# Westlake-AGI-Lab/WorldForge

Measured on AMD Instinct MI355X. Metric: denoising steps/sec (81f x 480p, Wan2.1-14B), higher is better.
Workload: dtype bf16

## Files before the change

### include/wf_hip.h

```cpp
#ifndef WF_HIP_H_
#define WF_HIP_H_

#include <stddef.h>
#include <stdint.h>

#ifdef __cplusplus
extern "C" {
#endif

#define WF_OK 0
#define WF_EINVAL (-1)
#define WF_EHIP (-2)
#define WF_ENOTSUP (-3)

#define WF_F32 0
#define WF_BF16 1

int wf_version(void);
const char* wf_last_error(void);
int wf_device_info(int dev, int* n_cu, int* clock_khz, char* name, int name_len);


int wf_cfg_combine(const void* cond, const void* uncond, void* out, int dt, float g, size_t n, void* stream);

// ... 57 lines not shown
int wf_gemm_f16_batched(const void* X, const void* W, void* out, int batch, int M, int N, int K, int ldx, int ldw, int ldo, int64_t bsx,
                        int64_t bsw, int64_t bso, int epilogue, void* stream);
int wf_mx_quant_e4m3(const void* X, void* Q, void* S, int M, int K, int ldx, void* stream);
int wf_gemm_mxfp8(const void* Xq, const void* Xs, const void* Wq, const void* Ws, const float* bias, void* out, const float* gate, int M, int N,
                  int K, int ldx, int ldw, int ldo, int epilogue, void* stream);
int wf_lora_fold(const void* base, void* out, int N, int K, int n_adapters, const void* U0, const void* D0, int rank0, int nsep0,
                 float scale0, const void* U1, const void* D1, int rank1, int nsep1, float scale1, const void* U2, const void* D2,
                 int rank2, int nsep2, float scale2, const void* U3, const void* D3, int rank3, int nsep3, float scale3, void* stream);

int wf_attn_fwd(const void* Q, const void* K, const void* Vt, void* O, int H, int Lq, int Lkp, int kv_len, int seg_len,
                size_t seg_stride_bytes, int ldo, float softmax_scale, int accumulate, const float* kmax2, int kmax_n, int kmax_stride,
                const float* qmax2, int qmax_n, void* stream);
int wf_head_max_norm2(const void* X, int H, int L, int Lp, float* out, void* stream);
size_t wf_attn_split_workspace_bytes(int H, int Lq, int nsplit);
int wf_attn_cross2_fwd(const void* Q, const void* K, const void* Vt, void* O, int H, int Lq, int Lk1p, int kv_len1, int Lk2p, int kv_len2,
                       int ldo, float softmax_scale, void* stream);
int wf_attn_debug_body_counter(void* counters2);
int wf_attn_fwd_split(const void* Q, const void* K, const void* Vt, void* O, int H, int Lq, int Lkp, int kv_len, int seg_len,
                      size_t seg_stride_bytes, int ldo, float softmax_scale, int accumulate, int nsplit, void* workspace, const float* kmax2,
                      int kmax_n, int kmax_stride, const float* qmax2, int qmax_n, void* stream);
int wf_attn_fwd_part(const void* Q, const void* K, const void* Vt, int H, int Lq, int Lkp, int kv_len, int seg_len, size_t seg_stride_bytes,
                     int t_begin, int t_end, int t_begin2, int t_end2, int inner_splits, int part, int nparts, void* workspace, void* O_merge,
                     int ldo, const float* kmax2, int kmax_n, int kmax_stride, const float* qmax2, int qmax_n, void* stream);
int wf_attn_merge(void* O, int H, int Lq, int ldo, int accumulate, int nparts, const void* workspace, void* stream);

int wf_ln_modulate(const float* x, const float* mul, const float* add, void* out, int out_dtype, int L, int C, float eps,
                   int plus_one, void* stream);

int wf_rmsnorm_heads(const void* in, int ld, const float* weight, const float* cos_tab, const float* sin_tab, void* out, int L,
                     int Lout, int C, float eps, float out_scale, void* stream);
size_t wf_rmsnorm_heads_bound_ws_floats(int L, int C);
int wf_rmsnorm_heads_bound(const void* in, int ld, const float* weight, const float* cos_tab, const float* sin_tab, void* out, int L, int Lout,
                           int C, float eps, float out_scale, float* ws, float* max_norm2, void* stream);

int wf_v_transpose(const void* V, int ld, void* Vt, int L, int Lp, int H, void* stream);
int wf_v_transpose_seg(const void* V, int ld, void* Vt, int L, int Lp, int H, int head_stride_tiles, void* stream);
int wf_v_transpose_at(const void* V, int ld, void* Vt, int k0, int L, int Lp, int H, void* stream);

int wf_patchify(const void* x, void* tokens, int Cin, int T, int Hh, int Ww, void* stream);
int wf_unpatchify(const float* y, float* out, int Cout, int T, int Hh, int Ww, void* stream);

int wf_act(const void* a, int dt_a, const void* b, int dt_b, void* out, int dt_out, int mode, size_t n, void* stream);

int wf_lc_ln_modulate(const void* x, const float* mul, const float* add, int64_t mod_ld, int rows_per_group, int64_t row0,
                      const int* group_index, int plus_one, void* out, int L, int C, float eps, void* stream);
int wf_lc_gate_residual(void* x, const void* y, int64_t ldy, const float* gate, int64_t gate_ld, int rows_per_group, int64_t row0,
                        const int* group_index, int L, int C, void* stream);
int wf_lc_norm_heads(const void* in, int64_t ld, const float* weight, const float* cos_tab, const float* sin_tab, void* out, int L,
                     int Lout, int H, float eps, float out_scale, void* stream);
int wf_lc_swiglu(const void* in, int64_t ld, void* out, int L, int Hd, void* stream);

int wf_refine_upsample_u8(const void* frames_u8, float* out, int F, int H0, int W0, int Fo, int H, int W, void* stream);

int wf_lc_mean_pool_blocks(const void* in, void* out, int H, int L, int block, void* stream);
int wf_lc_mean_pool_blocks_at(const void* in, int64_t in_head_stride_rows, void* out, int out_head_stride_blocks, int b0, int H, int L,
                              int block, void* stream);
int wf_bsa_topk_lists(const void* scores, int64_t ld, int heads, int n_q, int n_k, int n_sel, int block, int blocks_per_segment,
                      int* lists, int* counts, int max_entries, uint32_t* sel_mask, void* stream);
int wf_bsa_cdf_lists(const void* scores, int64_t ld, int heads, int n_q, int n_k, float cdf_threshold, int n_min, int block,
                     int blocks_per_segment, int* lists, int* counts, int max_entries, uint32_t* sel_mask, int* row_counts, void* stream);
int wf_gather_rows_bf16(const void* in, int64_t ld_in, const int* index, void* out, int64_t ld_out, int n_rows, int C, void* stream);
int wf_attn_bsa_fwd(const void* Q, const void* K, const void* Vt, void* O, int H, int Lq, int Lkp, int seg_len, int ldo,
                    float softmax_scale, const int* group_lists, const int* group_counts, int max_entries, int block, void* stream);

int wf_t5_attn_fwd(const void* Q, const void* K, const void* V, int ldqkv, void* O, int ldo, const float* bias, const void* bucket_lut,
                   int lmax, int num_buckets, int H, int L, int kv_len, void* stream);
// ... 122 lines not shown
```

### worldforge_amd/csrc/dit_ops.hip

```cpp
#include "common.h"
#include "mfma.h"

using namespace wf;

namespace {

__device__ __forceinline__ float block_sum_1(float v, float* sm, int nwaves) {
  v = wave_sum(v);
  const int lane = threadIdx.x & 63, wid = threadIdx.x >> 6;
  __syncthreads();
  if (lane == 0) sm[wid] = v;
  __syncthreads();
  float t = 0.f;
  for (int i = 0; i < nwaves; ++i) t += sm[i];
  return t;
}

template <int VPT>
__global__ __launch_bounds__(256) void k_ln_mod(const float* __restrict__ x, const float* __restrict__ mul,
                                                const float* __restrict__ add, void* __restrict__ out, int out_bf16, int C,
                                                float eps, float plus_one) {
  __shared__ float sm[8];
  const size_t row = blockIdx.x;
  const float4* xr = reinterpret_cast<const float4*>(x + row * C);
  const int nvec = C >> 2;
  float4 v[VPT];
  float s = 0.f;
#pragma unroll
  for (int i = 0; i < VPT; ++i) {
    int id = threadIdx.x + 256 * i;
    if (id < nvec) {
      v[i] = xr[id];
      s += (v[i].x + v[i].y) + (v[i].z + v[i].w);
    } else {
      v[i] = make_float4(0.f, 0.f, 0.f, 0.f);
    }
  }
  const float mean = block_sum_1(s, sm, 4) / (float)C;
  float q = 0.f;
#pragma unroll
  for (int i = 0; i < VPT; ++i) {
    int id = threadIdx.x + 256 * i;
    if (id < nvec) {
      float a = v[i].x - mean, b = v[i].y - mean, c = v[i].z - mean, d = v[i].w - mean;
      q += (a * a + b * b) + (c * c + d * d);
    }
  }
  const float var = block_sum_1(q, sm, 4) / (float)C;
  const float rstd = rsqrtf(var + eps);
#pragma unroll
  for (int i = 0; i < VPT; ++i) {
    int id = threadIdx.x + 256 * i;
    if (id < nvec) {
      float4 m4 = mul ? reinterpret_cast<const float4*>(mul)[id] : make_float4(0.f, 0.f, 0.f, 0.f);
      float4 a4 = add ? reinterpret_cast<const float4*>(add)[id] : make_float4(0.f, 0.f, 0.f, 0.f);
      float y0 = (v[i].x - mean) * rstd * (plus_one + m4.x) + a4.x;
      float y1 = (v[i].y - mean) * rstd * (plus_one + m4.y) + a4.y;
      float y2 = (v[i].z - mean) * rstd * (plus_one + m4.z) + a4.z;
      float y3 = (v[i].w - mean) * rstd * (plus_one + m4.w) + a4.w;
      if (out_bf16) {
        u32x2 pk = {pack_bf16x2(y0, y1), pack_bf16x2(y2, y3)};
        reinterpret_cast<u32x2*>(reinterpret_cast<uint16_t*>(out) + row * C)[id] = pk;
      } else {
        reinterpret_cast<float4*>(reinterpret_cast<float*>(out) + row * C)[id] = make_float4(y0, y1, y2, y3);
      }
    }
  }
}

__global__ __launch_bounds__(128) void k_rms_heads(const uint16_t* __restrict__ in, int ld, const float* __restrict__ w,
                                                   const float* __restrict__ cs, const float* __restrict__ sn,
                                                   uint16_t* __restrict__ out, int L, int Lout, int C, float eps, float out_scale,
                                                   float* __restrict__ norm2_rows) {
  __shared__ float sm[4];
  const int row = blockIdx.x;
  const uint16_t* xr = in + (size_t)row * ld;
  const int nch = C >> 3;
  constexpr int MAXC = 8;
  u32x4 v[MAXC];
  float ss = 0.f;
#pragma unroll
  for (int i = 0; i < MAXC; ++i) {
    int id = threadIdx.x + 128 * i;
    if (id < nch) {
      v[i] = reinterpret_cast<const u32x4*>(xr)[id];
#pragma unroll
      for (int k = 0; k < 4; ++k) {
        float a = __uint_as_float(v[i][k] << 16), b = __uint_as_float(v[i][k] & 0xffff0000u);
        ss += a * a + b * b;
      }
    }
  }
  const float tot = block_sum_1(ss, sm, 2);
  const float rinv = rsqrtf(tot / (float)C + eps);
  const int H = C >> 7;
#pragma unroll
  for (int i = 0; i < MAXC; ++i) {
    int id = threadIdx.x + 128 * i;
    if (id < nch) {
      const int head = id >> 4, within = id & 15;
      const float4 w0 = reinterpret_cast<const float4*>(w)[2 * id], w1 = reinterpret_cast<const float4*>(w)[2 * id + 1];
      const float ww[8] = {w0.x, w0.y, w0.z, w0.w, w1.x, w1.y, w1.z, w1.w};
      float y[8];
#pragma unroll
      for (int k = 0; k < 4; ++k) {
        float a = __uint_as_float(v[i][k] << 16), b = __uint_as_float(v[i][k] & 0xffff0000u);
        y[2 * k] = rbf(rbf(a * rinv) * ww[2 * k]);
        y[2 * k + 1] = rbf(rbf(b * rinv) * ww[2 * k + 1]);
      }
      if (cs) {
        const float4 c4 = reinterpret_cast<const float4*>(cs + (size_t)row * 64)[within];
        const float4 s4 = reinterpret_cast<const float4*>(sn + (size_t)row * 64)[within];
        const float cc[4] = {c4.x, c4.y, c4.z, c4.w}, sv[4] = {s4.x, s4.y, s4.z, s4.w};
#pragma unroll
        for (int k = 0; k < 4; ++k) {
          float re = y[2 * k] * cc[k] - y[2 * k + 1] * sv[k];
          float im = y[2 * k] * sv[k] + y[2 * k + 1] * cc[k];
          y[2 * k] = re;
          y[2 * k + 1] = im;
        }
      }
      if (out_scale != 1.0f) {
#pragma unroll
        for (int k = 0; k < 8; ++k) y[k] *= out_scale;
      }
      u32x4 pk = {pack_bf16x2(y[0], y[1]), pack_bf16x2(y[2], y[3]), pack_bf16x2(y[4], y[5]), pack_bf16x2(y[6], y[7])};
      *reinterpret_cast<u32x4*>(out + ((size_t)head * Lout + row) * 128 + within * 8) = pk;
      if (norm2_rows) {
        float q = 0.f;
#pragma unroll
        for (int k = 0; k < 4; ++k) {
          const float a = __uint_as_float(pk[k] << 16), b = __uint_as_float(pk[k] & 0xffff0000u);
          q += a * a + b * b;
        }
        q += __shfl_xor(q, 8, 64);
        q += __shfl_xor(q, 4, 64);
        q += __shfl_xor(q, 2, 64);
        q += __shfl_xor(q, 1, 64);
        if (within == 0) norm2_rows[(size_t)row * H + head] = q;
      }
    }
  }
}

constexpr int NB_RB = 128;
__device__ __forceinline__ float nb_max(float best, float v) { return !(v <= 3.0e38f) ? INFINITY : fmaxf(best, v); }
__device__ __forceinline__ float nb_column_max(const float* __restrict__ src, int n, int H, int h, int s, int ns) {
  float best = 0.f;
  int r = s;
  for (; r + 7 * ns < n; r += 8 * ns) {
    float v[8];
#pragma unroll
    for (int u = 0; u < 8; ++u) v[u] = src[(size_t)(r + u * ns) * H + h];
#pragma unroll
    for (int u = 0; u < 8; ++u) best = nb_max(best, v[u]);
  }
  for (; r < n; r += ns) best = nb_max(best, src[(size_t)r * H + h]);
  return best;
}
__global__ __launch_bounds__(256) void k_norm2_part(const float* __restrict__ rows, int L, int H, float* __restrict__ part) {
  __shared__ float red[256];
  const int t = threadIdx.x, h = t % H, s = t / H, ns = 256 / H;
  const int r0 = blockIdx.x * NB_RB, n = min(L - r0, NB_RB);
  float best = s < ns ? nb_column_max(rows + (size_t)r0 * H, n, H, h, s, ns) : 0.f;
  red[t] = best;
  __syncthreads();
  if (t < H) {
    for (int k = 1; k < ns; ++k) best = fmaxf(best, red[k * H + t]);
    part[(size_t)blockIdx.x * H + t] = best;
  }
}
__global__ __launch_bounds__(256) void k_norm2_final(const float* __restrict__ part, int nblk, int H, float* __restrict__ out) {
  __shared__ float red[256];
  const int t = threadIdx.x, h = t % H, s = t / H, ns = 256 / H;
  float best = s < ns ? nb_column_max(part, nblk, H, h, s, ns) : 0.f;
// ... 2 lines not shown
  if (t < H) {
    for (int k = 1; k < ns; ++k) best = fmaxf(best, red[k * H + t]);
    out[t] = best;
  }
}

__global__ __launch_bounds__(256) void k_vt(const uint16_t* __restrict__ V, int ld, uint16_t* __restrict__ Vt, int L, int hstride) {
  __shared__ uint16_t tile[64][136];
  const int kt = blockIdx.x, head = blockIdx.y;
  const int tid = threadIdx.x;
#pragma unroll
  for (int i = 0; i < 4; ++i) {
    int id = tid + 256 * i;
    int r = id >> 4, c = id & 15;
    int key = kt * 64 + r;
    u32x4 v = {0u, 0u, 0u, 0u};
    if (key < L) v = *reinterpret_cast<const u32x4*>(V + (size_t)key * ld + head * 128 + c * 8);
    *reinterpret_cast<u32x4*>(&tile[r][c * 8]) = v;
  }
  __syncthreads();
  uint16_t* dst = Vt + ((size_t)head * hstride + kt) * (128 * 64);
#pragma unroll
  for (int i = 0; i < 4; ++i) {
    int id = tid + 256 * i;
    int d = id >> 3, c = id & 7;
    uint32_t p[4];
#pragma unroll
    for (int k = 0; k < 4; ++k) p[k] = (uint32_t)tile[c * 8 + 2 * k][d] | ((uint32_t)tile[c * 8 + 2 * k + 1][d] << 16);
    u32x4 pk = {p[0], p[1], p[2], p[3]};
    *reinterpret_cast<u32x4*>(dst + d * 64 + c * 8) = pk;
  }
}

__global__ void k_patchify(const uint16_t* __restrict__ x, uint16_t* __restrict__ out, int Cin, int T, int Hh, int Ww, size_t n) {
  const int h2 = Hh >> 1, w2 = Ww >> 1, K = Cin * 4;
  for (size_t i = (size_t)blockIdx.x * blockDim.x + threadIdx.x; i < n; i += (size_t)gridDim.x * blockDim.x) {
    int k = (int)(i % K);
    size_t tok = i / K;
    int c = k >> 2, ph = (k >> 1) & 1, pw = k & 1;
    int wx = (int)(tok % w2), hy = (int)((tok / w2) % h2), f = (int)(tok / ((size_t)w2 * h2));
    out[i] = x[(((size_t)c * T + f) * Hh + (2 * hy + ph)) * Ww + (2 * wx + pw)];
  }
}
__global__ void k_unpatchify(const float* __restrict__ y, float* __restrict__ out, int Cout, int T, int Hh, int Ww, size_t n) {
  const int h2 = Hh >> 1, w2 = Ww >> 1;
  for (size_t i = (size_t)blockIdx.x * blockDim.x + threadIdx.x; i < n; i += (size_t)gridDim.x * blockDim.x) {
    int xw = (int)(i % Ww), yh = (int)((i / Ww) % Hh), f = (int)((i / ((size_t)Ww * Hh)) % T), c = (int)(i / ((size_t)Ww * Hh * T));
    size_t tok = ((size_t)f * h2 + (yh >> 1)) * w2 + (xw >> 1);
    int k = (((yh & 1) << 1) | (xw & 1)) * Cout + c;
    out[i] = y[tok * (4 * Cout) + k];
  }
}

__global__ void k_act(TView a, TView b, TView o, int mode, size_t n) {
  for (size_t i = (size_t)blockIdx.x * blockDim.x + threadIdx.x; i < n; i += (size_t)gridDim.x * blockDim.x) {
    float v = tload(a, i);
    if (b.p) v += tload(b, i);
    if (mode == 0)
      v = v / (1.0f + __expf(-v));
    else if (mode == 1)
      v = 0.5f * v * (1.0f + erff(v * 0.70710678118654752f));
    tstore(o, i, v);
  }
}

}

extern "C" int wf_ln_modulate(const float* x, const float* mul, const float* add, void* out, int out_dtype, int L, int C,
                              float eps, int plus_one, void* stream) {
  WF_CHECK_ARG(x && out, "wf_ln_modulate: null pointer");
  WF_CHECK_ARG(C % 4 == 0 && C <= 8192 && C > 0, "wf_ln_modulate: C=%d must be a multiple of 4 and <= 8192", C);
  if (L == 0) return WF_OK;
  hipStream_t s = (hipStream_t)stream;
  const float p1 = plus_one ? 1.0f : 0.0f;
  const int ob = out_dtype == WF_BF16;
  const int nvec = C / 4;
  if (nvec <= 512)
    hipLaunchKernelGGL(k_ln_mod<2>, dim3(L), dim3(256), 0, s, x, mul, add, out, ob, C, eps, p1);
  else if (nvec <= 1280)
    hipLaunchKernelGGL(k_ln_mod<5>, dim3(L), dim3(256), 0, s, x, mul, add, out, ob, C, eps, p1);
  else
    hipLaunchKernelGGL(k_ln_mod<8>, dim3(L), dim3(256), 0, s, x, mul, add, out, ob, C, eps, p1);
  WF_LAUNCH_CHECK("wf_ln_modulate");
  return WF_OK;
}

extern "C" int wf_rmsnorm_heads(const void* in, int ld, const float* weight, const float* cos_tab, const float* sin_tab,
                                void* out, int L, int Lout, int C, float eps, float out_scale, void* stream) {
  WF_CHECK_ARG(in && weight && out, "wf_rmsnorm_heads: null pointer");
  WF_CHECK_ARG(out_scale > 0.0f, "wf_rmsnorm_heads: out_scale must be positive (1 = none)");
  WF_CHECK_ARG(C % 128 == 0 && C <= 8192 && ld % 8 == 0, "wf_rmsnorm_heads: C=%d must be a multiple of 128 (<= 8192), ld %% 8", C);
  WF_CHECK_ARG(Lout >= L, "wf_rmsnorm_heads: Lout < L");
  WF_CHECK_ARG((cos_tab == nullptr) == (sin_tab == nullptr), "wf_rmsnorm_heads: cos/sin must both be given or both null");
  if (L == 0) return WF_OK;
  hipLaunchKernelGGL(k_rms_heads, dim3(L), dim3(128), 0, (hipStream_t)stream, (const uint16_t*)in, ld, weight, cos_tab,
                     sin_tab, (uint16_t*)out, L, Lout, C, eps, out_scale, (float*)nullptr);
  WF_LAUNCH_CHECK("wf_rmsnorm_heads");
  return WF_OK;
}

extern "C" size_t wf_rmsnorm_heads_bound_ws_floats(int L, int C) {
  if (L <= 0 || C <= 0) return 0;
  const size_t H = (size_t)C / 128;
  return (size_t)L * H + (size_t)((L + NB_RB - 1) / NB_RB) * H;
}

extern "C" int wf_rmsnorm_heads_bound(const void* in, int ld, const float* weight, const float* cos_tab, const float* sin_tab, void* out,
                                      int L, int Lout, int C, float eps, float out_scale, float* ws, float* max_norm2, void* stream) {
  WF_CHECK_ARG(in && weight && out && ws && max_norm2, "wf_rmsnorm_heads_bound: null pointer");
  WF_CHECK_ARG(out_scale > 0.0f, "wf_rmsnorm_heads_bound: out_scale must be positive (1 = none)");
  WF_CHECK_ARG(C >= 128 && C % 128 == 0 && C <= 8192 && ld % 8 == 0, "wf_rmsnorm_heads_bound: C=%d must be a multiple of 128 in 128..8192, ld %% 8", C);
  WF_CHECK_ARG(Lout >= L && L > 0, "wf_rmsnorm_heads_bound: need 0 < L <= Lout");
  WF_CHECK_ARG((cos_tab == nullptr) == (sin_tab == nullptr), "wf_rmsnorm_heads_bound: cos/sin must both be given or both null");
  const int H = C / 128, nblk = (L + NB_RB - 1) / NB_RB;
  float* rows = ws;
  float* part = ws + (size_t)L * H;
  hipLaunchKernelGGL(k_rms_heads, dim3(L), dim3(128), 0, (hipStream_t)stream, (const uint16_t*)in, ld, weight, cos_tab,
                     sin_tab, (uint16_t*)out, L, Lout, C, eps, out_scale, rows);
  hipLaunchKernelGGL(k_norm2_part, dim3(nblk), dim3(256), 0, (hipStream_t)stream, rows, L, H, part);
  hipLaunchKernelGGL(k_norm2_final, dim3(1), dim3(256), 0, (hipStream_t)stream, part, nblk, H, max_norm2);
  WF_LAUNCH_CHECK("wf_rmsnorm_heads_bound");
  return WF_OK;
}

extern "C" int wf_v_transpose(const void* V, int ld, void* Vt, int L, int Lp, int H, void* stream) {
  WF_CHECK_ARG(V && Vt, "wf_v_transpose: null pointer");
  WF_CHECK_ARG(Lp % 64 == 0 && Lp >= L && ld % 8 == 0, "wf_v_transpose: Lp must be a multiple of 64 and >= L");
  if (Lp == 0) return WF_OK;
  hipLaunchKernelGGL(k_vt, dim3(Lp / 64, H), dim3(256), 0, (hipStream_t)stream, (const uint16_t*)V, ld, (uint16_t*)Vt, L, Lp / 64);
  WF_LAUNCH_CHECK("wf_v_transpose");
  return WF_OK;
}

extern "C" int wf_v_transpose_seg(const void* V, int ld, void* Vt, int L, int Lp, int H, int head_stride_tiles, void* stream) {
  WF_CHECK_ARG(V && Vt, "wf_v_transpose_seg: null pointer");
  WF_CHECK_ARG(Lp % 64 == 0 && Lp >= L && ld % 8 == 0, "wf_v_transpose_seg: Lp must be a multiple of 64 and >= L");
  WF_CHECK_ARG(head_stride_tiles >= Lp / 64, "wf_v_transpose_seg: head stride (%d tiles) shorter than the segment (%d)", head_stride_tiles, Lp / 64);
  if (Lp == 0) return WF_OK;
  hipLaunchKernelGGL(k_vt, dim3(Lp / 64, H), dim3(256), 0, (hipStream_t)stream, (const uint16_t*)V, ld, (uint16_t*)Vt, L, head_stride_tiles);
  WF_LAUNCH_CHECK("wf_v_transpose_seg");
  return WF_OK;
}

extern "C" int wf_patchify(const void* x, void* tokens, int Cin, int T, int Hh, int Ww, void* stream) {
  WF_CHECK_ARG(x && tokens, "wf_patchify: null pointer");
  WF_CHECK_ARG(Hh % 2 == 0 && Ww % 2 == 0, "wf_patchify: latent H, W must be even");
  size_t n = (size_t)T * (Hh / 2) * (Ww / 2) * Cin * 4;
  if (n == 0) return WF_OK;
  hipLaunchKernelGGL(k_patchify, dim3(grid_for(n, 256, 4096)), dim3(256), 0, (hipStream_t)stream, (const uint16_t*)x,
                     (uint16_t*)tokens, Cin, T, Hh, Ww, n);
  WF_LAUNCH_CHECK("wf_patchify");
  return WF_OK;
}

// ... 20 lines not shown
```

### worldforge_amd/dit.py

```python
from __future__ import annotations

import math
import os
from dataclasses import dataclass
from types import SimpleNamespace
from typing import Dict, Optional, Tuple

import numpy as np
import torch

from . import _ffi, ops
from ._ffi import WF_BF16, WF_F32, call
from .forward_common import (ForwardWorkspaces, GatheredLayerKV, act, bf16_latents, gather_layer_kv, layers_per_rank, run,
                             seeded_generators)

EPI_BF16, EPI_BF16_GELU, EPI_F32, EPI_RESID, EPI_F32_ACC = 0, 1, 2, 3, 4


@dataclass
class DiTConfig:
    dim: int = 5120
    ffn_dim: int = 13824
    num_heads: int = 40
    num_layers: int = 40
# ... 52 lines not shown
    out = dict(W)
    for k, v in W.items():
        if k.endswith(tuple(suffixes)):
            out[k] = MXWeight.quantize(v)
    return out


def gemm(x: torch.Tensor, w, bias: Optional[torch.Tensor], out: torch.Tensor, epi: int,
         gate: Optional[torch.Tensor] = None):
    if isinstance(w, MXWeight):
        xq, xs = _mx_act(x)
        return ops.gemm_mxfp8(xq, xs, w.q, w.s, bias, out, epi, gate)
    M, K = x.shape
    N = w.shape[0]
    assert w.shape[1] == K and x.dtype == torch.bfloat16 and w.dtype == torch.bfloat16
    assert out.shape[0] == M and out.shape[1] == N
    call("wf_gemm_bf16", x.data_ptr(), w.data_ptr(), bias.data_ptr() if bias is not None else None, out.data_ptr(),
         gate.data_ptr() if gate is not None else None, M, N, K, x.stride(0), w.stride(0), out.stride(0), epi, ops.stream())
    return out


def ffn_padded_features(f: int) -> int:
    fp = -(-f // 320) * 320
    return fp if (fp - f) * 100 <= 3 * f else f


def _pad_rows(t: torch.Tensor, rows: int) -> torch.Tensor:
    if t.shape[0] == rows:
        return t
    pad = torch.zeros((rows - t.shape[0],) + tuple(t.shape[1:]), dtype=t.dtype, device=t.device)
    return torch.cat([t, pad], 0).contiguous()


PROFILE_ATTN = None
PROFILE_COMM = None


def comm_wait_ms(entry) -> float:
    if isinstance(entry, list):
        return sum(a.elapsed_time(b) for a, b in entry)
    return entry[0].elapsed_time(entry[1])


def kv_splits(H: int, Lq: int, kv_len: int, n_cu: int = 256) -> int:
    if kv_len < 128 * 64:
        return 1
    w = -(-Lq // 256) * H
    eff = lambda n: (w * n / n_cu) / -(-(w * n) // n_cu)
    return 2 if eff(2) > eff(1) + 0.08 else 1


def head_max_norm2(k: torch.Tensor, L: int, out: torch.Tensor) -> torch.Tensor:
    H, Lp, _ = k.shape
    out.zero_()
    call("wf_head_max_norm2", k.data_ptr(), H, L, Lp, out.data_ptr(), ops.stream())
    return out


def attention(q: torch.Tensor, k: torch.Tensor, vt: torch.Tensor, out: torch.Tensor, kv_len: int, scale: float,
              accumulate: bool = False, profile: bool = False, nsplit: Optional[int] = None, kmax2: Optional[torch.Tensor] = None,
              qmax2: Optional[torch.Tensor] = None):
    H, Lq, D = q.shape
    seg_stride = 0
    if k.dim() == 4:
        P, _, seg, _ = k.shape
        assert vt.shape == (P, H, seg // 64, 128, 64)
# ... 595 lines not shown
        ws.hbuf = _buf("h", (L, d), bf)
        ws.qkv = _buf("qkv", (L, 3 * d), bf)
        ws.qh = _buf("qh", (H, L, 128), bf)
        ws.qm = _buf("qmax2", (H,), f32) if pl.use_bounds else None
        if pl.exchange is not None:
            ws.ex = self._exchange(pl.tag, H, Sp, pl.exchange, int(self.exchange_chunks))
        else:
            ws.kh = _buf("kh", (H, Sp, 128), bf, zero=True)
            ws.vt = _buf("vt", (H, Sp // 64, 128, 64), bf)
            ws.km = _buf("kmax2", (H,), f32) if pl.use_bounds else None
        ws.ao = _buf("ao", (L, d), bf)
        ws.qc = _buf("qc", (L, d), bf)
        ws.ffh = _buf("ffh", (L, ffn_padded_features(cfg.ffn_dim)), bf)
        ws.Lt, ws.Li = cfg.text_len, _pad64(n_img)
        ws.Lc = ws.Li + ws.Lt
        ws.kvt = _buf("kvt", (cfg.text_len, 2 * d), bf)
        ws.kvi = _buf("kvi", (n_img, 2 * d), bf)
        ws.kc = _buf("kc", (H, ws.Lc, 128), bf, zero=True)
        ws.vtc = _buf("vtc", (H, ws.Lc // 64, 128, 64), bf)
        ws.emod = _buf("emod", (6, d), f32)
        return ws

    def _prompt_context(self, pl, ws, emb, text, img) -> _PromptContext:
        return _PromptContext(self, pl, ws, emb, self._context_kv(text, img))

    def _sa_queries(self, pl, ws, i):
        self._heads(ws.qkv, 0, self._wl[f"blocks.{i}.self_attn.norm_q"], pl.cos, pl.sin, ws.qh, pl.L, out_scale=pl.q_scale, bound=ws.qm)

    def _sa_keys(self, pl, ws, i, r0, r1, kh, vt, km):
        d = self.cfg.dim
        self._heads(ws.qkv[r0:r1], d, self._wl[f"blocks.{i}.self_attn.norm_k"], pl.cos[r0:r1], pl.sin[r0:r1], kh, r1 - r0, bound=km)
        self._vt(ws.qkv[r0:r1], 2 * d, vt, r1 - r0)

    def _sa_local(self, pl, ws, i):
        W, p = self._wl, f"blocks.{i}."
        gemm(ws.hbuf, W[p + "qkv.w"], W[p + "qkv.b"], ws.qkv, EPI_BF16)
        self._sa_queries(pl, ws, i)
        self._sa_keys(pl, ws, i, 0, pl.L, ws.kh, ws.vt, ws.km)
        attention(ws.qh, ws.kh, ws.vt, ws.ao, pl.L, pl.sa_scale, profile=True, kmax2=ws.km, qmax2=ws.qm)

    def _sa_exchange(self, pl, ws, ctx, i):
        W, p, d, ex = self._wl, f"blocks.{i}.", self.cfg.dim, ws.ex
        gemm(ws.hbuf, W[p + "qkv.w"][d:], W[p + "qkv.b"][d:], ws.qkv[:, d:], EPI_BF16)
        for g in range(ex.G):
            r0, r1 = ex.chunk_rows(g, pl.L)
            if r1 > r0:
                self._sa_keys(pl, ws, i, r0, r1, ex.own_k(g), ex.own_vt(g), ex.own_km(g) if pl.use_bounds else None)
        ex.launch()
        if i == 0:
            ctx.launch_shared()
        yield i
        gemm(ws.hbuf, W[p + "qkv.w"][:d], W[p + "qkv.b"][:d], ws.qkv[:, :d], EPI_BF16)
        self._sa_queries(pl, ws, i)
        attention_exchange(ws.qh, ex, ws.ao, pl.L_tok, pl.sa_scale, ws.qm, use_bounds=pl.use_bounds, profile=True)

    def _sa_consume(self, pl, ctx, x, share):
        if pl.exchange is not None:
            ctx.launch_shared()
            yield 0
        x.copy_(share["x"])

    def _cross_attention(self, pl, ws, emb, ctx, i):
        W, p, x = self._wl, f"blocks.{i}.", emb.x
        self._ln(x, W[p + "norm3.w"], W[p + "norm3.b"], ws.hbuf, self.cfg.eps, plus_one=False)
        gemm(ws.hbuf, W[p + "cross_attn.q.w"], W[p + "cross_attn.q.b"], ws.qc, EPI_BF16)
        self._heads(ws.qc, 0, W[p + "cross_attn.norm_q"], None, None, ws.qh, pl.L)
        kc, vtc = ctx.layer(i)
        cross_attention2(ws.qh, kc, vtc, ws.ao, ws.Li, emb.n_img, ws.Lt, pl.scale)
        gemm(ws.ao, W[p + "cross_attn.o.w"], W[p + "cross_attn.o.b"], x, EPI_RESID, gate=None)

    def _ffn(self, ws, emb, i):
# ... 46 lines not shown
```

Measured before the change: 0.2388.

## Fuse Q/K RMSNorm+RoPE and V transpose into one kernel; wave-per-row norms

Adds a single wf_qkv_post kernel whose grid roles handle Q norm+RoPE, K norm+RoPE and the V transpose for self-attention. Before, these ran as three separate launches. LayerNorm-modulate and the RMS-head kernels are rewritten to map one row per wave, looping over several rows with register prefetch and warp-only reductions. Modulation vectors are staged in LDS. The aim is fewer launches and block-level syncs and better latency hiding on these memory-bound ops, at the cost of more registers and specialised template paths.

```diff
diff --git a/include/wf_hip.h b/include/wf_hip.h
--- a/include/wf_hip.h
+++ b/include/wf_hip.h
@@ -113,6 +113,10 @@
 size_t wf_rmsnorm_heads_bound_ws_floats(int L, int C);
 int wf_rmsnorm_heads_bound(const void* in, int ld, const float* weight, const float* cos_tab, const float* sin_tab, void* out, int L, int Lout,
                            int C, float eps, float out_scale, float* ws, float* max_norm2, void* stream);
+
+int wf_qkv_post(const void* qkv, int ld, const float* q_weight, const float* k_weight, const float* cos_tab, const float* sin_tab,
+                void* qh, void* kh, void* vt, int L, int Lq_out, int Lk_out, int Lp, int C, float eps, float q_scale, float* q_ws,
+                float* q_max_norm2, float* k_ws, float* k_max_norm2, void* stream);
 
 int wf_v_transpose(const void* V, int ld, void* Vt, int L, int Lp, int H, void* stream);
 int wf_v_transpose_seg(const void* V, int ld, void* Vt, int L, int Lp, int H, int head_stride_tiles, void* stream);
diff --git a/worldforge_amd/csrc/dit_ops.hip b/worldforge_amd/csrc/dit_ops.hip
--- a/worldforge_amd/csrc/dit_ops.hip
+++ b/worldforge_amd/csrc/dit_ops.hip
@@ -5,142 +5,216 @@
 
 namespace {
 
-__device__ __forceinline__ float block_sum_1(float v, float* sm, int nwaves) {
-  v = wave_sum(v);
-  const int lane = threadIdx.x & 63, wid = threadIdx.x >> 6;
+constexpr int RW_WAVES = 4;
+__device__ __forceinline__ int rw_wave() { return __builtin_amdgcn_readfirstlane((int)(threadIdx.x >> 6)); }
+static inline int rw_rows_per_wave(int L) {
+  const int r = ceil_div(L, 4096);
+  return r < 1 ? 1 : (r > 8 ? 8 : r);
+}
+__device__ __forceinline__ void lds_bar() {
+  asm volatile("s_waitcnt lgkmcnt(0)" ::: "memory");
+  __builtin_amdgcn_s_barrier();
+}
+
+template <int NJ, bool EX>
+__device__ __forceinline__ void ln_load(float4 (&v)[NJ], const float* __restrict__ x, int row, int C, int lane) {
+  const float4* xr = reinterpret_cast<const float4*>(x + (size_t)row * C) + lane;
+  const int nvec = C >> 2;
+#pragma unroll
+  for (int j = 0; j < NJ; ++j) {
+    if (EX || lane + 64 * j < nvec) v[j] = xr[64 * j];
+  }
+}
+
+template <int NJ, bool PF, bool EX>
+__global__ __launch_bounds__(256, 2) void k_ln_mod(const float* __restrict__ x, const float* __restrict__ mul,
+                                                   const float* __restrict__ add, void* __restrict__ out, int out_bf16, int L, int C,
+                                                   float eps, float plus_one, int rows_per_wave) {
+  __shared__ float4 s_pm[64 * NJ], s_add[64 * NJ];
+  const int nvec = C >> 2, lane = threadIdx.x & 63;
+  for (int id = threadIdx.x; id < nvec; id += 256) {
+    const float4 m4 = mul ? reinterpret_cast<const float4*>(mul)[id] : make_float4(0.f, 0.f, 0.f, 0.f);
+    s_pm[id] = make_float4(plus_one + m4.x, plus_one + m4.y, plus_one + m4.z, plus_one + m4.w);
+    s_add[id] = add ? reinterpret_cast<const float4*>(add)[id] : make_float4(0.f, 0.f, 0.f, 0.f);
+  }
   __syncthreads();
-  if (lane == 0) sm[wid] = v;
-  __syncthreads();
-  float t = 0.f;
-  for (int i = 0; i < nwaves; ++i) t += sm[i];
-  return t;
-}
-
-template <int VPT>
-__global__ __launch_bounds__(256) void k_ln_mod(const float* __restrict__ x, const float* __restrict__ mul,
-                                                const float* __restrict__ add, void* __restrict__ out, int out_bf16, int C,
-                                                float eps, float plus_one) {
-  __shared__ float sm[8];
-  const size_t row = blockIdx.x;
-  const float4* xr = reinterpret_cast<const float4*>(x + row * C);
-  const int nvec = C >> 2;
-  float4 v[VPT];
-  float s = 0.f;
-#pragma unroll
-  for (int i = 0; i < VPT; ++i) {
-    int id = threadIdx.x + 256 * i;
-    if (id < nvec) {
-      v[i] = xr[id];
-      s += (v[i].x + v[i].y) + (v[i].z + v[i].w);
+  const int base = blockIdx.x * (RW_WAVES * rows_per_wave), row_end = min(L, base + RW_WAVES * rows_per_wave);
+  const int row0 = base + rw_wave();
+  if (row0 >= row_end) return;
+  float4 v[NJ], nx[NJ];
+  if constexpr (PF) ln_load<NJ, EX>(nx, x, row0, C, lane);
+#pragma unroll 1
+  for (int row = row0; row < row_end; row += RW_WAVES) {
+    asm volatile("" ::: "memory");
+    if constexpr (PF) {
+#pragma unroll
+      for (int j = 0; j < NJ; ++j) v[j] = nx[j];
+      ln_load<NJ, EX>(nx, x, min(row + RW_WAVES, row_end - 1), C, lane);
     } else {
-      v[i] = make_float4(0.f, 0.f, 0.f, 0.f);
-    }
-  }
-  const float mean = block_sum_1(s, sm, 4) / (float)C;
-  float q = 0.f;
-#pragma unroll
-  for (int i = 0; i < VPT; ++i) {
-    int id = threadIdx.x + 256 * i;
-    if (id < nvec) {
-      float a = v[i].x - mean, b = v[i].y - mean, c = v[i].z - mean, d = v[i].w - mean;
-      q += (a * a + b * b) + (c * c + d * d);
-    }
-  }
-  const float var = block_sum_1(q, sm, 4) / (float)C;
-  const float rstd = rsqrtf(var + eps);
-#pragma unroll
-  for (int i = 0; i < VPT; ++i) {
-    int id = threadIdx.x + 256 * i;
-    if (id < nvec) {
-      float4 m4 = mul ? reinterpret_cast<const float4*>(mul)[id] : make_float4(0.f, 0.f, 0.f, 0.f);
-      float4 a4 = add ? reinterpret_cast<const float4*>(add)[id] : make_float4(0.f, 0.f, 0.f, 0.f);
-      float y0 = (v[i].x - mean) * rstd * (plus_one + m4.x) + a4.x;
-      float y1 = (v[i].y - mean) * rstd * (plus_one + m4.y) + a4.y;
-      float y2 = (v[i].z - mean) * rstd * (plus_one + m4.z) + a4.z;
-      float y3 = (v[i].w - mean) * rstd * (plus_one + m4.w) + a4.w;
-      if (out_bf16) {
-        u32x2 pk = {pack_bf16x2(y0, y1), pack_bf16x2(y2, y3)};
-        reinterpret_cast<u32x2*>(reinterpret_cast<uint16_t*>(out) + row * C)[id] = pk;
-      } else {
-        reinterpret_cast<float4*>(reinterpret_cast<float*>(out) + row * C)[id] = make_float4(y0, y1, y2, y3);
+      ln_load<NJ, EX>(v, x, row, C, lane);
+    }
+    float s[4] = {0.f, 0.f, 0.f, 0.f};
+#pragma unroll
+    for (int j = 0; j < NJ; ++j) {
+      if (EX || lane + 64 * j < nvec) s[j & 3] += (v[j].x + v[j].y) + (v[j].z + v[j].w);
+    }
+    float t = 0.f;
+#pragma unroll
+    for (int k = 0; k < 4; ++k) t += wave_sum(s[k]);
+    const float mean = t / (float)C;
+    float q[4] = {0.f, 0.f, 0.f, 0.f};
+#pragma unroll
+    for (int j = 0; j < NJ; ++j) {
+      if (EX || lane + 64 * j < nvec) {
+        float a = v[j].x - mean, b = v[j].y - mean, c = v[j].z - mean, d = v[j].w - mean;
+        q[j & 3] += (a * a + b * b) + (c * c + d * d);
+        v[j] = make_float4(a, b, c, d);
       }
     }
-  }
-}
-
-__global__ __launch_bounds__(128) void k_rms_heads(const uint16_t* __restrict__ in, int ld, const float* __restrict__ w,
-                                                   const float* __restrict__ cs, const float* __restrict__ sn,
-                                                   uint16_t* __restrict__ out, int L, int Lout, int C, float eps, float out_scale,
-                                                   float* __restrict__ norm2_rows) {
-  __shared__ float sm[4];
-  const int row = blockIdx.x;
-  const uint16_t* xr = in + (size_t)row * ld;
-  const int nch = C >> 3;
-  constexpr int MAXC = 8;
-  u32x4 v[MAXC];
-  float ss = 0.f;
-#pragma unroll
-  for (int i = 0; i < MAXC; ++i) {
-    int id = threadIdx.x + 128 * i;
-    if (id < nch) {
-      v[i] = reinterpret_cast<const u32x4*>(xr)[id];
-#pragma unroll
-      for (int k = 0; k < 4; ++k) {
-        float a = __uint_as_float(v[i][k] << 16), b = __uint_as_float(v[i][k] & 0xffff0000u);
-        ss += a * a + b * b;
+    t = 0.f;
+#pragma unroll
+    for (int k = 0; k < 4; ++k) t += wave_sum(q[k]);
+    const float var = t / (float)C;
+    const float rstd = rsqrtf(var + eps);
+#pragma unroll
+    for (int j = 0; j < NJ; ++j) {
+      const int id = lane + 64 * j;
+      if (EX || id < nvec) {
+        const float4 pm = s_pm[id], a4 = s_add[id];
+        float y0 = v[j].x * rstd * pm.x + a4.x;
+        float y1 = v[j].y * rstd * pm.y + a4.y;
+        float y2 = v[j].z * rstd * pm.z + a4.z;
+        float y3 = v[j].w * rstd * pm.w + a4.w;
+        if (out_bf16) {
+          u32x2 pk = {pack_bf16x2(y0, y1), pack_bf16x2(y2, y3)};
+          reinterpret_cast<u32x2*>(reinterpret_cast<uint16_t*>(out) + (size_t)row * C)[id] = pk;
+        } else {
+          reinterpret_cast<float4*>(reinterpret_cast<float*>(out) + (size_t)row * C)[id] = make_float4(y0, y1, y2, y3);
+        }
       }
     }
   }
-  const float tot = block_sum_1(ss, sm, 2);
-  const float rinv = rsqrtf(tot / (float)C + eps);
-  const int H = C >> 7;
-#pragma unroll
-  for (int i = 0; i < MAXC; ++i) {
-    int id = threadIdx.x + 128 * i;
-    if (id < nch) {
-      const int head = id >> 4, within = id & 15;
-      const float4 w0 = reinterpret_cast<const float4*>(w)[2 * id], w1 = reinterpret_cast<const float4*>(w)[2 * id + 1];
-      const float ww[8] = {w0.x, w0.y, w0.z, w0.w, w1.x, w1.y, w1.z, w1.w};
-      float y[8];
-#pragma unroll
-      for (int k = 0; k < 4; ++k) {
-        float a = __uint_as_float(v[i][k] << 16), b = __uint_as_float(v[i][k] & 0xffff0000u);
-        y[2 * k] = rbf(rbf(a * rinv) * ww[2 * k]);
-        y[2 * k + 1] = rbf(rbf(b * rinv) * ww[2 * k + 1]);
+}
+
+struct RmsArgs {
+  const uint16_t* in;
+  int ld;
+  const float* w;
+  const float *cs, *sn;
+  uint16_t* out;
+  int Lout, C;
+  float eps, out_scale;
+  float* norm2_rows;
+};
+template <int CPL>
+struct RmsRow {
+  u32x4 v[CPL];
+  float4 c4, s4;
+};
+template <int CPL, bool EX>
+__device__ __forceinline__ void rms_load(RmsRow<CPL>& r, const RmsArgs& a, int row, int lane) {
+  const u32x4* xr = reinterpret_cast<const u32x4*>(a.in + (size_t)row * a.ld) + lane;
+  const int nch = a.C >> 3;
+#pragma unroll
+  for (int j = 0; j < CPL; ++j) {
+    if (EX || lane + 64 * j < nch) r.v[j] = xr[64 * j];
+  }
+  if (a.cs) {
+    r.c4 = reinterpret_cast<const float4*>(a.cs + (size_t)row * 64)[lane & 15];
+    r.s4 = reinterpret_cast<const float4*>(a.sn + (size_t)row * 64)[lane & 15];
+  }
+}
+
+template <int CPL, bool PF, bool EX>
+__device__ __forceinline__ void rms_walk(const RmsArgs& a, int row0, int row_end) {
+  if (row0 >= row_end) return;
+  const int lane = threadIdx.x & 63, within = lane & 15;
+  const int nch = a.C >> 3, H = a.C >> 7, C = a.C;
+  const float out_scale = a.out_scale;
+  const size_t hstep = (size_t)a.Lout * (4 * 128);
+  uint16_t* const olane = a.out + (size_t)(lane >> 4) * a.Lout * 128 + within * 8;
+  float4 w0[CPL], w1[CPL];
+#pragma unroll
+  for (int j = 0; j < CPL; ++j) {
+    if (EX || lane + 64 * j < nch) {
+      w0[j] = reinterpret_cast<const float4*>(a.w)[2 * (lane + 64 * j)];
+      w1[j] = reinterpret_cast<const float4*>(a.w)[2 * (lane + 64 * j) + 1];
+    }
+  }
+  RmsRow<CPL> cur, nxt;
+  if constexpr (PF) rms_load<CPL, EX>(nxt, a, row0, lane);
+#pragma unroll 1
+  for (int row = row0; row < row_end; row += RW_WAVES) {
+    if constexpr (PF) {
+      cur = nxt;
+      rms_load<CPL, EX>(nxt, a, min(row + RW_WAVES, row_end - 1), lane);
+    } else {
+      rms_load<CPL, EX>(cur, a, row, lane);
+    }
+    float ss[2] = {0.f, 0.f};
+#pragma unroll
+    for (int j = 0; j < CPL; ++j) {
+      if (EX || lane + 64 * j < nch) {
+#pragma unroll
+        for (int k = 0; k < 4; ++k) {
+          float x0 = __uint_as_float(cur.v[j][k] << 16), x1 = __uint_as_float(cur.v[j][k] & 0xffff0000u);
+          ss[j & 1] += x0 * x0 + x1 * x1;
+        }
       }
-      if (cs) {
-        const float4 c4 = reinterpret_cast<const float4*>(cs + (size_t)row * 64)[within];
-        const float4 s4 = reinterpret_cast<const float4*>(sn + (size_t)row * 64)[within];
-        const float cc[4] = {c4.x, c4.y, c4.z, c4.w}, sv[4] = {s4.x, s4.y, s4.z, s4.w};
+    }
+    float tot = 0.f;
+    tot += wave_sum(ss[0]);
+    tot += wave_sum(ss[1]);
+    const float rinv = rsqrtf(tot / (float)C + a.eps);
+#pragma unroll
+    for (int j = 0; j < CPL; ++j) {
+      if (EX || lane + 64 * j < nch) {
+        const float ww[8] = {w0[j].x, w0[j].y, w0[j].z, w0[j].w, w1[j].x, w1[j].y, w1[j].z, w1[j].w};
+        float y[8];
 #pragma unroll
         for (int k = 0; k < 4; ++k) {
-          float re = y[2 * k] * cc[k] - y[2 * k + 1] * sv[k];
-          float im = y[2 * k] * sv[k] + y[2 * k + 1] * cc[k];
-          y[2 * k] = re;
-          y[2 * k + 1] = im;
+          float x0 = __uint_as_float(cur.v[j][k] << 16), x1 = __uint_as_float(cur.v[j][k] & 0xffff0000u);
+          y[2 * k] = rbf(rbf(x0 * rinv) * ww[2 * k]);
+          y[2 * k + 1] = rbf(rbf(x1 * rinv) * ww[2 * k + 1]);
+        }
+        if (a.cs) {
+          const float cc[4] = {cur.c4.x, cur.c4.y, cur.c4.z, cur.c4.w}, sv[4] = {cur.s4.x, cur.s4.y, cur.s4.z, cur.s4.w};
+#pragma unroll
+          for (int k = 0; k < 4; ++k) {
+            float re = y[2 * k] * cc[k] - y[2 * k + 1] * sv[k];
+            float im = y[2 * k] * sv[k] + y[2 * k + 1] * cc[k];
+            y[2 * k] = re;
+            y[2 * k + 1] = im;
+          }
+        }
+        if (out_scale != 1.0f) {
+#pragma unroll
+          for (int k = 0; k < 8; ++k) y[k] *= out_scale;
+        }
+        u32x4 pk = {pack_bf16x2(y[0], y[1]), pack_bf16x2(y[2], y[3]), pack_bf16x2(y[4], y[5]), pack_bf16x2(y[6], y[7])};
+        *reinterpret_cast<u32x4*>(olane + j * hstep + (size_t)row * 128) = pk;
+        if (a.norm2_rows) {
+          float q = 0.f;
+#pragma unroll
+          for (int k = 0; k < 4; ++k) {
+            const float p0 = __uint_as_float(pk[k] << 16), p1 = __uint_as_float(pk[k] & 0xffff0000u);
+            q += p0 * p0 + p1 * p1;
+          }
+          q += __shfl_xor(q, 8, 64);
+          q += __shfl_xor(q, 4, 64);
+          q += __shfl_xor(q, 2, 64);
+          q += __shfl_xor(q, 1, 64);
+          if (within == 0) a.norm2_rows[(size_t)row * H + (lane >> 4) + 4 * j] = q;
         }
       }
-      if (out_scale != 1.0f) {
-#pragma unroll
-        for (int k = 0; k < 8; ++k) y[k] *= out_scale;
-      }
-      u32x4 pk = {pack_bf16x2(y[0], y[1]), pack_bf16x2(y[2], y[3]), pack_bf16x2(y[4], y[5]), pack_bf16x2(y[6], y[7])};
-      *reinterpret_cast<u32x4*>(out + ((size_t)head * Lout + row) * 128 + within * 8) = pk;
-      if (norm2_rows) {
-        float q = 0.f;
-#pragma unroll
-        for (int k = 0; k < 4; ++k) {
-          const float a = __uint_as_float(pk[k] << 16), b = __uint_as_float(pk[k] & 0xffff0000u);
-          q += a * a + b * b;
-        }
-        q += __shfl_xor(q, 8, 64);
-        q += __shfl_xor(q, 4, 64);
-        q += __shfl_xor(q, 2, 64);
-        q += __shfl_xor(q, 1, 64);
-        if (within == 0) norm2_rows[(size_t)row * H + head] = q;
-      }
-    }
-  }
+    }
+  }
+}
+
+template <int CPL, bool PF, bool EX>
+__global__ __launch_bounds__(256, EX ? 2 : 1) void k_rms_heads(RmsArgs a, int L, int rows_per_wave) {
+  const int base = blockIdx.x * (RW_WAVES * rows_per_wave);
+  rms_walk<CPL, PF, EX>(a, base + rw_wave(), min(L, base + RW_WAVES * rows_per_wave));
 }
 
 constexpr int NB_RB = 128;
@@ -209,6 +283,70 @@
   }
 }
 
+constexpr int VT_HB = 2;
+struct QkvPostArgs {
+  RmsArgs q, k;
+  const uint16_t* V;
+  uint16_t* Vt;
+  int L, H;
+};
+__device__ __forceinline__ void vt_load(u32x4 (&v)[VT_HB][4], const QkvPostArgs& a, int ld, int kt, int h0) {
+#pragma unroll
+  for (int b = 0; b < VT_HB; ++b) {
+#pragma unroll
+    for (int i = 0; i < 4; ++i) {
+      const int id = threadIdx.x + 256 * i;
+      const int r = id >> 4, c = id & 15;
+      const int key = kt * 64 + r;
+      u32x4 t = {0u, 0u, 0u, 0u};
+      if (key < a.L && h0 + b < a.H) t = *reinterpret_cast<const u32x4*>(a.V + (size_t)key * ld + (h0 + b) * 128 + c * 8);
+      v[b][i] = t;
+    }
+  }
+}
+template <int CPL, bool PF, bool EX>
+__global__ __launch_bounds__(256, EX ? 2 : 1) void k_qkv_post(QkvPostArgs a) {
+  __shared__ uint16_t tile[VT_HB][64][136];
+  const int role = blockIdx.x, kt = blockIdx.y;
+  if (role < 2) {
+    const int base = kt * 64;
+    rms_walk<CPL, PF, EX>(role == 0 ? a.q : a.k, base + rw_wave(), min(a.L, base + 64));
+    return;
+  }
+  const int tid = threadIdx.x, ld = a.q.ld, hstride = gridDim.y;
+  u32x4 v[VT_HB][4];
+  vt_load(v, a, ld, kt, 0);
+  for (int h0 = 0; h0 < a.H; h0 += VT_HB) {
+#pragma unroll
+    for (int b = 0; b < VT_HB; ++b) {
+#pragma unroll
+      for (int i = 0; i < 4; ++i) {
+        const int id = tid + 256 * i;
+        *reinterpret_cast<u32x4*>(&tile[b][id >> 4][(id & 15) * 8]) = v[b][i];
+      }
+    }
+    if (h0 + VT_HB < a.H) vt_load(v, a, ld, kt, h0 + VT_HB);
+    lds_bar();
+#pragma unroll
+    for (int b = 0; b < VT_HB; ++b) {
+      if (h0 + b < a.H) {
+        uint16_t* dst = a.Vt + ((size_t)(h0 + b) * hstride + kt) * (128 * 64);
+#pragma unroll
+        for (int i = 0; i < 4; ++i) {
+          const int id = tid + 256 * i;
+          const int d = id >> 3, c = id & 7;
+          uint32_t p[4];
+#pragma unroll
+          for (int k = 0; k < 4; ++k) p[k] = (uint32_t)tile[b][c * 8 + 2 * k][d] | ((uint32_t)tile[b][c * 8 + 2 * k + 1][d] << 16);
+          u32x4 pk = {p[0], p[1], p[2], p[3]};
+          *reinterpret_cast<u32x4*>(dst + d * 64 + c * 8) = pk;
+        }
+      }
+    }
+    lds_bar();
+  }
+}
+
 __global__ void k_patchify(const uint16_t* __restrict__ x, uint16_t* __restrict__ out, int Cin, int T, int Hh, int Ww, size_t n) {
   const int h2 = Hh >> 1, w2 = Ww >> 1, K = Cin * 4;
   for (size_t i = (size_t)blockIdx.x * blockDim.x + threadIdx.x; i < n; i += (size_t)gridDim.x * blockDim.x) {
@@ -252,14 +390,44 @@
   const float p1 = plus_one ? 1.0f : 0.0f;
   const int ob = out_dtype == WF_BF16;
   const int nvec = C / 4;
-  if (nvec <= 512)
-    hipLaunchKernelGGL(k_ln_mod<2>, dim3(L), dim3(256), 0, s, x, mul, add, out, ob, C, eps, p1);
+  const int rpw = rw_rows_per_wave(L);
+  const dim3 grid(ceil_div(L, RW_WAVES * rpw));
+#define WF_LN_CALL(NJ, PF, EX) hipLaunchKernelGGL((k_ln_mod<NJ, PF, EX>), grid, dim3(256), 0, s, x, mul, add, out, ob, L, C, eps, p1, rpw)
+  if (C == 5120)
+    WF_LN_CALL(20, true, true);
+  else if (C == 1536)
+    WF_LN_CALL(6, true, true);
+  else if (nvec <= 512)
+    WF_LN_CALL(8, true, false);
   else if (nvec <= 1280)
-    hipLaunchKernelGGL(k_ln_mod<5>, dim3(L), dim3(256), 0, s, x, mul, add, out, ob, C, eps, p1);
+    WF_LN_CALL(20, true, false);
   else
-    hipLaunchKernelGGL(k_ln_mod<8>, dim3(L), dim3(256), 0, s, x, mul, add, out, ob, C, eps, p1);
+    WF_LN_CALL(32, false, false);
+#undef WF_LN_CALL
   WF_LAUNCH_CHECK("wf_ln_modulate");
   return WF_OK;
+}
+
+#define WF_RMS_DISPATCH(C, CALL)     \
+  do {                               \
+    if ((C) == 5120) {               \
+      CALL(10, true, true);          \
+    } else if ((C) == 1536) {        \
+      CALL(3, true, true);           \
+    } else if ((C) <= 2048) {        \
+      CALL(4, true, false);          \
+    } else if ((C) <= 5120) {        \
+      CALL(10, true, false);         \
+    } else {                         \
+      CALL(16, false, false);        \
+    }                                \
+  } while (0)
+static void launch_rms_heads(const RmsArgs& a, int L, hipStream_t s) {
+  const int rpw = rw_rows_per_wave(L);
+  const dim3 grid(ceil_div(L, RW_WAVES * rpw));
+#define WF_RMS_CALL(CPL, PF, EX) hipLaunchKernelGGL((k_rms_heads<CPL, PF, EX>), grid, dim3(256), 0, s, a, L, rpw)
+  WF_RMS_DISPATCH(a.C, WF_RMS_CALL);
+#undef WF_RMS_CALL
 }
 
 extern "C" int wf_rmsnorm_heads(const void* in, int ld, const float* weight, const float* cos_tab, const float* sin_tab,
@@ -270,8 +438,8 @@
   WF_CHECK_ARG(Lout >= L, "wf_rmsnorm_heads: Lout < L");
   WF_CHECK_ARG((cos_tab == nullptr) == (sin_tab == nullptr), "wf_rmsnorm_heads: cos/sin must both be given or both null");
   if (L == 0) return WF_OK;
-  hipLaunchKernelGGL(k_rms_heads, dim3(L), dim3(128), 0, (hipStream_t)stream, (const uint16_t*)in, ld, weight, cos_tab,
-                     sin_tab, (uint16_t*)out, L, Lout, C, eps, out_scale, (float*)nullptr);
+  launch_rms_heads(RmsArgs{(const uint16_t*)in, ld, weight, cos_tab, sin_tab, (uint16_t*)out, Lout, C, eps, out_scale, nullptr}, L,
+                   (hipStream_t)stream);
   WF_LAUNCH_CHECK("wf_rmsnorm_heads");
   return WF_OK;
 }
@@ -292,11 +460,49 @@
   const int H = C / 128, nblk = (L + NB_RB - 1) / NB_RB;
   float* rows = ws;
   float* part = ws + (size_t)L * H;
-  hipLaunchKernelGGL(k_rms_heads, dim3(L), dim3(128), 0, (hipStream_t)stream, (const uint16_t*)in, ld, weight, cos_tab,
-                     sin_tab, (uint16_t*)out, L, Lout, C, eps, out_scale, rows);
+  launch_rms_heads(RmsArgs{(const uint16_t*)in, ld, weight, cos_tab, sin_tab, (uint16_t*)out, Lout, C, eps, out_scale, rows}, L,
+                   (hipStream_t)stream);
   hipLaunchKernelGGL(k_norm2_part, dim3(nblk), dim3(256), 0, (hipStream_t)stream, rows, L, H, part);
   hipLaunchKernelGGL(k_norm2_final, dim3(1), dim3(256), 0, (hipStream_t)stream, part, nblk, H, max_norm2);
   WF_LAUNCH_CHECK("wf_rmsnorm_heads_bound");
+  return WF_OK;
+}
+
+extern "C" int wf_qkv_post(const void* qkv, int ld, const float* q_weight, const float* k_weight, const float* cos_tab,
+                           const float* sin_tab, void* qh, void* kh, void* vt, int L, int Lq_out, int Lk_out, int Lp, int C, float eps,
+                           float q_scale, float* q_ws, float* q_max_norm2, float* k_ws, float* k_max_norm2, void* stream) {
+  WF_CHECK_ARG(qkv && q_weight && k_weight && qh && kh && vt, "wf_qkv_post: null pointer");
+  WF_CHECK_ARG(q_scale > 0.0f, "wf_qkv_post: q_scale must be positive (1 = none)");
+  WF_CHECK_ARG(C >= 128 && C % 128 == 0 && C <= 8192 && ld % 8 == 0 && ld >= 3 * C,
+               "wf_qkv_post: C=%d must be a multiple of 128 in 128..8192, ld %% 8, ld >= 3 C", C);
+  WF_CHECK_ARG(L > 0 && Lq_out >= L && Lk_out >= L && Lp >= L && Lp % 64 == 0, "wf_qkv_post: need 0 < L <= Lq_out, Lk_out, Lp and Lp %% 64 == 0");
+  WF_CHECK_ARG((cos_tab == nullptr) == (sin_tab == nullptr), "wf_qkv_post: cos/sin must both be given or both null");
+  WF_CHECK_ARG((q_ws == nullptr) == (q_max_norm2 == nullptr) && (k_ws == nullptr) == (k_max_norm2 == nullptr),
+               "wf_qkv_post: a bound needs both its workspace and its output");
+  WF_CHECK_ARG(q_ws == nullptr || q_ws != k_ws, "wf_qkv_post: the two bounds need separate workspaces");
+  hipStream_t s = (hipStream_t)stream;
+  const uint16_t* x = (const uint16_t*)qkv;
+  const int H = C / 128, nblk = (L + NB_RB - 1) / NB_RB;
+  QkvPostArgs a;
+  a.q = RmsArgs{x, ld, q_weight, cos_tab, sin_tab, (uint16_t*)qh, Lq_out, C, eps, q_scale, q_ws};
+  a.k = RmsArgs{x + C, ld, k_weight, cos_tab, sin_tab, (uint16_t*)kh, Lk_out, C, eps, 1.0f, k_ws};
+  a.V = x + 2 * (size_t)C;
+  a.Vt = (uint16_t*)vt;
+  a.L = L;
+  a.H = H;
+  const dim3 grid(3, Lp / 64);
+#define WF_QKV_CALL(CPL, PF, EX) hipLaunchKernelGGL((k_qkv_post<CPL, PF, EX>), grid, dim3(256), 0, s, a)
+  WF_RMS_DISPATCH(C, WF_QKV_CALL);
+#undef WF_QKV_CALL
+  if (q_ws) {
+    hipLaunchKernelGGL(k_norm2_part, dim3(nblk), dim3(256), 0, s, q_ws, L, H, q_ws + (size_t)L * H);
+    hipLaunchKernelGGL(k_norm2_final, dim3(1), dim3(256), 0, s, q_ws + (size_t)L * H, nblk, H, q_max_norm2);
+  }
+  if (k_ws) {
+    hipLaunchKernelGGL(k_norm2_part, dim3(nblk), dim3(256), 0, s, k_ws, L, H, k_ws + (size_t)L * H);
+    hipLaunchKernelGGL(k_norm2_final, dim3(1), dim3(256), 0, s, k_ws + (size_t)L * H, nblk, H, k_max_norm2);
+  }
+  WF_LAUNCH_CHECK("wf_qkv_post");
   return WF_OK;
 }
 
diff --git a/worldforge_amd/dit.py b/worldforge_amd/dit.py
--- a/worldforge_amd/dit.py
+++ b/worldforge_amd/dit.py
@@ -108,6 +108,7 @@
     return torch.cat([t, pad], 0).contiguous()
 
 
+SA_QKV_POST = True
 PROFILE_ATTN = None
 PROFILE_COMM = None
 
@@ -769,11 +770,26 @@
         self._heads(ws.qkv[r0:r1], d, self._wl[f"blocks.{i}.self_attn.norm_k"], pl.cos[r0:r1], pl.sin[r0:r1], kh, r1 - r0, bound=km)
         self._vt(ws.qkv[r0:r1], 2 * d, vt, r1 - r0)
 
+    def _sa_qkv_post(self, pl, ws, i):
+        cfg, W, p = self.cfg, self._wl, f"blocks.{i}.self_attn."
+        qws = kws = None
+        if pl.use_bounds:
+            n = int(_ffi.lib().wf_rmsnorm_heads_bound_ws_floats(pl.L, cfg.dim))
+            qws, kws = self._buf("heads_bound_ws", (n,), torch.float32), self._buf("heads_bound_ws_k", (n,), torch.float32)
+        ptr = lambda t: t.data_ptr() if t is not None else None
+        call("wf_qkv_post", ws.qkv.data_ptr(), ws.qkv.stride(0), W[p + "norm_q"].data_ptr(), W[p + "norm_k"].data_ptr(), pl.cos.data_ptr(),
+             pl.sin.data_ptr(), ws.qh.data_ptr(), ws.kh.data_ptr(), ws.vt.data_ptr(), pl.L, ws.qh.shape[1], ws.kh.shape[1],
+             ws.vt.shape[1] * 64, cfg.dim, float(cfg.eps), float(pl.q_scale), ptr(qws), ptr(ws.qm if pl.use_bounds else None), ptr(kws),
+             ptr(ws.km if pl.use_bounds else None), ops.stream())
+
     def _sa_local(self, pl, ws, i):
         W, p = self._wl, f"blocks.{i}."
         gemm(ws.hbuf, W[p + "qkv.w"], W[p + "qkv.b"], ws.qkv, EPI_BF16)
-        self._sa_queries(pl, ws, i)
-        self._sa_keys(pl, ws, i, 0, pl.L, ws.kh, ws.vt, ws.km)
+        if SA_QKV_POST:
+            self._sa_qkv_post(pl, ws, i)
+        else:
+            self._sa_queries(pl, ws, i)
+            self._sa_keys(pl, ws, i, 0, pl.L, ws.kh, ws.vt, ws.km)
         attention(ws.qh, ws.kh, ws.vt, ws.ao, pl.L, pl.sa_scale, profile=True, kmax2=ws.km, qmax2=ws.qm)
 
     def _sa_exchange(self, pl, ws, ctx, i):
```

New measurement: 0.2389, median of 5. No clear change (+0.0%).
